# tuna2134/sbv2-api

Measured on AMD Instinct MI355X. Metric: audio_seconds_per_second, higher is better.
Workload: dtype bf16x3-split (decoder + flow convs: bf16 hi/lo MFMA, f32 accumulate/storage) + f16x3 (DeBERTa GEMMs, flow 1x1: f16 hi + scaled f16 lo per operand, 22 mantissa bits, f32 accumulate) + f32 (text side)

## Files before the change

include/sbv2_hip.h:

```cpp
#ifndef SBV2_HIP_H
#define SBV2_HIP_H

#include <stddef.h>
#include <stdint.h>

#ifdef __cplusplus
extern "C" {
#endif

typedef struct sbv2_bert sbv2_bert;
typedef struct sbv2_vits sbv2_vits;
typedef struct sbv2_pipeline sbv2_pipeline;

const char* sbv2_last_error(void);
int sbv2_device_count(void);

int sbv2_bert_create(const uint8_t* model, size_t model_len, int device, sbv2_bert** out);
void sbv2_bert_destroy(sbv2_bert* h);
int64_t sbv2_bert_hidden(const sbv2_bert* h);
int sbv2_bert_gemm_parts(const sbv2_bert* h);

int sbv2_bert_predict(sbv2_bert* h, const int64_t* token_ids, const int64_t* attention_mask, int64_t S, float* out);
int sbv2_bert_predict_batch(sbv2_bert* h, int64_t n, const int64_t* token_ids, const int64_t* attention_mask,
                            const int64_t* lens, float* out);
// ... 354 lines not shown
                           float* ms);
int sbv2_debug_set_skinny_max(int workgroups);
int sbv2_debug_set_clx(int on);
int sbv2_debug_set_ksplit(int on);
int sbv2_debug_set_flash_parts(int on);
int sbv2_debug_conv1d_clx(int device, const float* x, const float* w, const float* bias, const float* res, int64_t cin, int64_t cout, int64_t k,
                          int64_t L, int64_t dilation, float pre_slope, float beta, int64_t iters, float* y, float* ys_sum, float* ms);
int sbv2_debug_f16x3_saturation(int device, int enable, uint64_t* count);
int sbv2_debug_set_respair_clx(int on);
int sbv2_debug_respair(int device, const float* x, const float* w1, const float* w2, const float* b1, const float* b2, int64_t C, int64_t N, int64_t k,
                       int64_t dilation, const uint8_t* mask, int64_t mask_div, float beta, int accumulate, int variant, float* y);
int sbv2_debug_set_resbranch(int on);
int sbv2_debug_set_upx(int on);
int sbv2_debug_conv_transpose1d_clx(int device, const float* x, const float* w, const float* bias, int64_t cin, int64_t cout, int64_t k, int64_t L,
                                    int64_t stride, float pre_slope, const uint8_t* mask, int64_t mask_div, int64_t iters, float* y, float* ys_sum, float* ms);
int sbv2_debug_resbranch(int device, const float* x, const float* w, const float* bias, int64_t C, int64_t N, int64_t k, const int64_t* dilations,
                         const uint8_t* mask, int64_t mask_div, float beta, int accumulate, int variant, int64_t iters, float* y, float* ms);
int sbv2_debug_resbranch_ys(int device, const float* x, const float* w, const float* bias, int64_t C, int64_t N, int64_t k, const int64_t* dilations,
                            const uint8_t* mask, int64_t mask_div, float beta, int accumulate, int64_t iters, float* y, float* ys, float* y_steps, float* ys_steps,
                            float* ms);
int sbv2_debug_gemm_bfs(int device, const float* x, const float* w, const float* bias, const float* res, int64_t M, int64_t N, int64_t K,
                        int parts, int act, int split_out, int64_t iters, float* y, float* ms);
int sbv2_debug_gemm_bfs_alt(int device, const float* xa, const float* xb, const float* w, const float* bias, const float* res, int64_t M, int64_t N, int64_t K,
                            int parts, int64_t iters, float* ya, float* yb);
int sbv2_debug_repeat_respair(int device, const float* xa, const float* xb, const float* w1, const float* w2, const float* b1, const float* b2, int64_t C,
                              int64_t N, int64_t k, int64_t dilation, const uint8_t* mask, int64_t mask_div, float beta, const float* prev, int variant,
                              int reps, int neighbour, int flip_at, int64_t flip_word, float* ya, float* yb, int64_t* mismatch, int64_t* first_bad);
int sbv2_debug_repeat_resbranch(int device, const float* xa, const float* xb, const float* w, const float* bias, int64_t C, int64_t N, int64_t k,
                                const int64_t* dilations, const uint8_t* mask, int64_t mask_div, float beta, const float* prev, int reps, int neighbour,
                                int flip_at, int64_t flip_word, float* ya, float* yb, int64_t* mismatch, int64_t* first_bad);
// ... 77 lines not shown
```

sbv2-api_amd/_lib.py:

```python
import ctypes as C
import os

_HERE = os.path.dirname(os.path.abspath(__file__))
LIB_PATH = os.path.join(_HERE, "libsbv2_hip.so")

i64p = C.POINTER(C.c_int64)
f32p = C.POINTER(C.c_float)


class Sbv2Batch(C.Structure):
    _fields_ = [
        ("n", C.c_int64), ("t_lens", i64p), ("x_tst", i64p), ("tones", i64p), ("lang_ids", i64p), ("sids", i64p),
        ("style_vectors", f32p), ("bert", f32p),
        ("sdp_ratio", C.c_float), ("length_scale", C.c_float), ("noise_scale", C.c_float), ("noise_scale_w", C.c_float),
        ("noise_seed", C.c_uint64), ("forced_durations", i64p),
    ]


class Sbv2PcmFormat(C.Structure):
    _fields_ = [("sample_rate", C.c_int32), ("encoding", C.c_int32), ("normalize", C.c_int32), ("reserved", C.c_int32)]


class Sbv2Loudness(C.Structure):
    _fields_ = [("target_lufs", C.c_double), ("true_peak_max_dbtp", C.c_double)]
# ... 253 lines not shown
    "sbv2_style_vector": (C.c_int, [f32p, C.c_int64, C.c_int64, C.c_int64, C.c_float, f32p]),
    "sbv2_debug_import_to_container": (C.c_int, [C.c_void_p, C.c_size_t, C.c_int, C.POINTER(C.c_void_p), C.POINTER(C.c_size_t)]),
    "sbv2_debug_bucket_table": (C.c_int, [C.c_int64, C.c_int64, C.c_int64, C.POINTER(C.c_int32)]),
    "sbv2_debug_conv1d": (C.c_int, [C.c_int, f32p, f32p, f32p, C.c_int64, C.c_int64, C.c_int64, C.c_int64, C.c_int64, C.c_float, f32p]),
    "sbv2_debug_conv_transpose1d": (C.c_int, [C.c_int, f32p, f32p, f32p, C.c_int64, C.c_int64, C.c_int64, C.c_int64, C.c_int64,
                                              C.c_int64, C.c_float, f32p]),
    "sbv2_debug_conv1d_cl": (C.c_int, [C.c_int, f32p, f32p, f32p, C.c_int64, C.c_int64, C.c_int64, C.c_int64, C.c_int64, C.c_float, C.c_int,
                                       C.c_int64, f32p, f32p]),
    "sbv2_debug_time_conv1d": (C.c_int, [C.c_int, C.c_int64, C.c_int64, C.c_int64, C.c_int64, C.c_int64, C.c_int64, f32p]),
    "sbv2_debug_set_skinny_max": (C.c_int, [C.c_int]),
    "sbv2_debug_set_clx": (C.c_int, [C.c_int]),
    "sbv2_debug_set_ksplit": (C.c_int, [C.c_int]),
    "sbv2_debug_set_flash_parts": (C.c_int, [C.c_int]),
    "sbv2_debug_conv1d_clx": (C.c_int, [C.c_int, f32p, f32p, f32p, f32p, C.c_int64, C.c_int64, C.c_int64, C.c_int64, C.c_int64, C.c_float, C.c_float,
                                        C.c_int64, f32p, f32p, f32p]),
    "sbv2_debug_set_respair_clx": (C.c_int, [C.c_int]),
    "sbv2_debug_f16x3_saturation": (C.c_int, [C.c_int, C.c_int, C.POINTER(C.c_uint64)]),
    "sbv2_debug_respair": (C.c_int, [C.c_int, f32p, f32p, f32p, f32p, f32p, C.c_int64, C.c_int64, C.c_int64, C.c_int64, C.c_void_p, C.c_int64, C.c_float, C.c_int,
                                     C.c_int, f32p]),
    "sbv2_debug_set_resbranch": (C.c_int, [C.c_int]),
    "sbv2_debug_set_upx": (C.c_int, [C.c_int]),
    "sbv2_debug_conv_transpose1d_clx": (C.c_int, [C.c_int, f32p, f32p, f32p, C.c_int64, C.c_int64, C.c_int64, C.c_int64, C.c_int64, C.c_float, C.c_void_p,
                                                  C.c_int64, C.c_int64, f32p, f32p, f32p]),
    "sbv2_debug_resbranch": (C.c_int, [C.c_int, f32p, f32p, f32p, C.c_int64, C.c_int64, C.c_int64, i64p, C.c_void_p, C.c_int64, C.c_float, C.c_int, C.c_int,
                                       C.c_int64, f32p, f32p]),
    "sbv2_debug_resbranch_ys": (C.c_int, [C.c_int, f32p, f32p, f32p, C.c_int64, C.c_int64, C.c_int64, i64p, C.c_void_p, C.c_int64, C.c_float, C.c_int,
                                          C.c_int64, f32p, f32p, f32p, f32p, f32p]),
    "sbv2_debug_gemm_bfs_alt": (C.c_int, [C.c_int, f32p, f32p, f32p, f32p, f32p, C.c_int64, C.c_int64, C.c_int64, C.c_int, C.c_int64, f32p, f32p]),
    "sbv2_debug_repeat_respair": (C.c_int, [C.c_int, f32p, f32p, f32p, f32p, f32p, f32p, C.c_int64, C.c_int64, C.c_int64, C.c_int64, C.c_void_p, C.c_int64,
                                            C.c_float, f32p, C.c_int, C.c_int, C.c_int, C.c_int, C.c_int64, f32p, f32p, i64p, i64p]),
# ... 78 lines not shown
```

sbv2-api_amd/csrc/common.h:

```cpp
#pragma once
#include <hip/hip_runtime.h>

#include <atomic>

#include <cstdint>
#include <cstdio>
#include <map>
#include <memory>
#include <stdexcept>
#include <exception>
#include <string>
#include <vector>

namespace sbv2 {

void set_last_error(const std::string& msg);

struct Error : std::runtime_error {
    using std::runtime_error::runtime_error;
};

#define HIP_CHECK(expr)                                                                          \
    do {                                                                                         \
        hipError_t _e = (expr);                                                                  \
// ... 253 lines not shown
    const unsigned char* mask = nullptr;
    int mask_div = 1;
    int out_stride = 1, phase_rows = 1 << 30;
    int phase_off[kMaxPhases] = {0};
    int in_km = 0, out_km = 0;
    int act = ACT_NONE;
    float alpha = 1.0f;
    void* ys_p = nullptr;
    int64_t ys_rows = 0;
    int ys_front = 0;
    float ys_slope = 1.0f;
};
void launch_conv_cl(const ConvClParams& p, hipStream_t stream);
bool conv_cl_parts_ok(const ConvClParams& p);
bool launch_conv_cl_small(const ConvClParams& p, int mask_shift, hipStream_t stream);

constexpr int kPartsF16x3 = 4;
constexpr float kF16LoScale = 2048.0f;
inline int split_nplanes(int code) { return code == kPartsF16x3 ? 2 : code; }
struct SplitPlanes {
    void* p = nullptr;
    int parts = 0, C = 0, L = 0, ld = 0;
    int f16 = 0;
    int64_t pstride = 0;
    unsigned long long* sat = nullptr;
    int code() const { return f16 ? kPartsF16x3 : parts; }
    SplitPlanes rows(int c0, int n) const {
        SplitPlanes s = *this;
        s.p = static_cast<char*>(p) + (size_t)c0 * ld * 2;
        s.C = n;
// ... 217 lines not shown
```

sbv2-api_amd/csrc/conv_clx.hip:

```cpp
#include <atomic>
#include <type_traits>

#include "common.h"
#include "device_prims.h"

#pragma clang fp contract(off)

namespace sbv2 {

constexpr int kClxNT = 256;
constexpr int kClxXR = 320;

struct ClxKernelParams {
    ConvClxParams p;
    int xrows;
    int wshift0;
    int sh0, sh_step;
    int gy;
};

template <int NTAPS, int kClxWR, int kClxXB, int XR, int EPI, bool PH = false>
__global__ __launch_bounds__(256) __attribute__((amdgpu_waves_per_eu(kClxWR * 4096 + kClxXB * 2 * XR * 32 <= 53 * 1024 ? 3 : 2))) void conv_clx_kernel(const ClxKernelParams kp) {
    constexpr bool EDGE = EPI == 1;
    static_assert(!PH || EPI == 0 || EPI == 3, "phased output: whole-tile channels-last epilogues only");
// ... 297 lines not shown
            int ostride = 1, mch = m;
            int64_t orow = nf16;
            if constexpr (PH) {
                ostride = p.out_stride;
                if (p.phase_group == 2) {
                    const int blk = (m0 >> 5) + i, nb = p.phase_rows >> 4;
                    const int pg = blk / nb;
                    mch = (blk - pg * nb) * 16 + (c8 & 15);
                    orow = (int64_t)nf16 * ostride + p.phase_off[2 * pg] + (c8 >> 4);
                } else {
                    const int ph = m0 / p.phase_rows;
                    mch = m - ph * p.phase_rows;
                    orow = (int64_t)nf16 * ostride + p.phase_off[ph];
                }
            }
            float* yp = p.Y ? p.Y + orow * p.ldy + mch : nullptr;
            const int64_t ystep = (int64_t)16 * ostride * p.ldy;
            const int64_t qstep = (int64_t)512 * ostride;
            char* qs = p.Ys.p ? static_cast<char*>(p.Ys.p) + ((int64_t)(mch >> 4) * 2) * yplane + ((int64_t)p.Ys.front + orow) * 32 + (mch & 15) * 2 : nullptr;
#pragma unroll
            for (int it = 0; it < 4; ++it) {
                f32x4v v[2];
#pragma unroll
                for (int h = 0; h < 2; ++h) {
                    const f32x4v a = *reinterpret_cast<const f32x4v*>(trow8 + it * 16 * 36 + 4 * h);
                    v[h] = a + b8[i][h];
                    if (p.R) v[h] += acc_y ? ld[0][it][h] : ld[i][it][h];
                    v[h] *= beta;
                    if (acc_y) v[h] += ld[1][it][h];
                    if (!allkeep && !((mbits >> it) & 1u)) v[h] = f32x4v{0.f, 0.f, 0.f, 0.f};
                }
// ... 32 lines not shown
        constexpr int i = decltype(ic)::value;
        tile_write(ic);
        const int m = m0 + i * 32 + c4;
        const f32x4v b4 = p.bias ? *reinterpret_cast<const f32x4v*>(p.bias + m) : f32x4v{0.f, 0.f, 0.f, 0.f};
#pragma unroll 1
        for (int it = 0; it < 8; ++it) {
            const int n = nfirst + it * 8;
            const int64_t pp = min(n, N - 1);
            const f32x4v a = *reinterpret_cast<const f32x4v*>(trow + it * 8 * 36);
            f32x4v v = a + b4;
            if (p.R) v += *reinterpret_cast<const f32x4v*>(p.R + pp * p.ldr + m);
            v *= beta;
            if (p.accumulate) v += *reinterpret_cast<const f32x4v*>(p.Y + pp * p.ldy + m);
            if (p.mask && !p.mask[pp >> p.mask_shift]) v = f32x4v{0.f, 0.f, 0.f, 0.f};
            if (n < N) {
                if (p.Y) *reinterpret_cast<f32x4v*>(p.Y + (int64_t)n * p.ldy + m) = v;
                if (p.Ys.p) {
                    char* qs = static_cast<char*>(p.Ys.p) + ((int64_t)(m >> 4) * 2) * yplane + ((int64_t)p.Ys.front + n) * 32 + (m & 15) * 2;
                    bf16x4 h, l;
#pragma unroll
                    for (int e = 0; e < 4; ++e) {
                        const float x = fmaxf(v[e], v[e] * sl);
                        h[e] = (__bf16)x;
                        l[e] = (__bf16)(x - (float)h[e]);
                    }
                    *reinterpret_cast<bf16x4*>(qs) = h;
                    *reinterpret_cast<bf16x4*>(qs + yplane) = l;
                }
            }
        }
    });
// ... 83 lines not shown
    hipLaunchKernelGGL(k_split_cl_km, dim3((unsigned)((x.L + 255) / 256), x.C >> 4), dim3(256), 0, stream, x.p, x.ld, (int64_t)x.L, x.C, slope, out);
    HIP_CHECK(hipGetLastError());
}

bool conv_clx_usable(const ConvClxParams& p) {
    if (!(p.ntaps == 3 || p.ntaps == 5 || p.ntaps == 7 || p.ntaps == 11 || (p.phase_rows && (p.ntaps == 2 || p.ntaps == 4)))) return false;
    if (p.Ykm && (p.Y || p.Ys.p || p.accumulate || p.R)) return false;
    if ((p.K & 31) || (p.M & 63) || p.K != p.X.C) return false;
    int tapmax = p.ntaps - 1;
    if (p.phase_rows)
        for (int q = 0; q < kMaxPhases && q < p.M / std::max(p.phase_rows, 1); ++q) tapmax = std::max(tapmax, p.ntaps - 1 + p.phase_tap0[q]);
    const int span = tapmax * std::abs(p.shift_step);
    if (span > kClxXR - kClxNT || p.shift0 < -kClxFront || p.shift0 + span > 64) return false;
    if (p.mask && p.mask_shift < 0) return false;
    if (p.Y && (p.ldy & 3)) return false;
    if (p.R && (p.ldr & 3)) return false;
    if (p.phase_rows) {
        if ((p.phase_rows & 63) || p.M % p.phase_rows || p.M / p.phase_rows > kMaxPhases || p.out_stride < 1 || p.R || p.accumulate || p.Ykm || p.N < kClxNT ||
            (p.ntaps & 1)) return false;
        if (p.Y && p.ldy < p.phase_rows) return false;
        if (p.Ys.p && (p.Ys.C != p.phase_rows || p.Ys.N != (int64_t)p.N * p.out_stride)) return false;
        for (int q = 0; q < p.M / p.phase_rows; ++q)
            if (p.phase_off[q] < 0 || p.phase_off[q] >= p.out_stride) return false;
        if (p.phase_group == 2) {
            if ((p.M / p.phase_rows) & 1) return false;
            for (int q = 0; q < p.M / p.phase_rows; q += 2)
                if (p.phase_off[q + 1] != p.phase_off[q] + 1 || p.phase_tap0[q + 1] != p.phase_tap0[q]) return false;
        } else if (p.phase_group != 1) return false;
        for (int q = 0; q < p.M / p.phase_rows; ++q)
            if (p.phase_tap0[q] < 0 || p.phase_tap0[q] > 8) return false;
// ... 104 lines not shown
```

sbv2-api_amd/csrc/decoder_cl.cpp:

```cpp
#include <algorithm>
#include <atomic>
#include <cmath>
#include <cstring>

#include "models.h"

namespace sbv2 {

static inline uint16_t f32_to_bf16_rne(float f) {
    uint32_t u;
    std::memcpy(&u, &f, 4);
    if ((u & 0x7FFFFFFFu) > 0x7F800000u) return (uint16_t)((u >> 16) | 0x40);
    u += 0x7FFFu + ((u >> 16) & 1u);
    return (uint16_t)(u >> 16);
}
static inline uint16_t f32_to_f16_rne(float f) {
    uint32_t u;
    std::memcpy(&u, &f, 4);
    const uint32_t sign = (u >> 16) & 0x8000u;
    u &= 0x7FFFFFFFu;
    if (u >= 0x7F800000u) return (uint16_t)(sign | 0x7C00u | (u > 0x7F800000u ? 0x200u : 0u));
    if (u >= 0x477FF000u) return (uint16_t)(sign | 0x7C00u);
    if (u < 0x33000001u) return (uint16_t)sign;
    int e = (int)(u >> 23) - 127;
// ... 154 lines not shown
    u.ntaps = U;
    u.shift0 = -tmin;
    u.nph = s;
    u.cout = cout;
    u.group = group;
    u.alg_macs_per_pos = macs;
    for (int r = 0; r < s; ++r) {
        u.phase_off[r] = r;
        u.phase_tap0[r] = t0[r] - tmin;
    }
    return u;
}

static int cl_parts_of(int mode) { return mode == 1 ? 2 : (mode == 2 ? 1 : 3); }

ClConv pack_decoder_conv(WeightStore& ws, const float* w, int M, int K, int k, int mode, const float* bias) {
    ClConv c = pack_cl(ws, w, M, K, k, cl_parts_of(mode), bias);
    if (mode == 1 && M == 16 && K == 16) c.wp = pack_cl_pairs(ws, w, k);
    return c;
}

void VitsModel::load_decoder_cl(const Blob& blob) {
    auto conv = [&](const std::string& prefix, int mode) {
        const HostTensor& t = blob.get(prefix + ".weight");
        const float* b = blob.has(prefix + ".bias") ? blob.get(prefix + ".bias").data : nullptr;
        return pack_decoder_conv(*ws_, t.data, (int)t.dims[0], (int)t.dims[1], (int)t.dims[2], mode, b);
    };
    std::vector<int> stage_mode(cfg_.up_rates.size(), dec_mode_);
    if (const char* e = getenv("SBV2_DECODER_STAGES")) {
        std::string v(e);
// ... 11 lines not shown
    }
    cl_pre_ = conv("dec.conv_pre", dec_mode_);
    int C = cfg_.up_initial;
    const int nk = (int)cfg_.res_kernels.size();
    for (size_t i = 0; i < cfg_.up_rates.size(); ++i) {
        ClStage st;
        st.mode = stage_mode[i];
        st.rate = cfg_.up_rates[i];
        st.cin = C;
        C /= 2;
        st.ch = C;
        const HostTensor& t = blob.get("dec.ups." + std::to_string(i) + ".weight");
        const float* ub = blob.get("dec.ups." + std::to_string(i) + ".bias").data;
        const int k = (int)t.dims[2], s = st.rate, pad = (k - s) / 2, cin = (int)t.dims[0], cout = (int)t.dims[1];
        SBV2_REQUIRE(k - 2 * pad == s, "transposed conv must upsample exactly by its stride");
        std::vector<std::vector<int>> tsets(s);
        for (int r = 0; r < s; ++r)
            for (int tt = -k; tt <= k; ++tt) {
                const int j = s * tt + r + pad;
                if (j >= 0 && j < k) tsets[r].push_back(tt);
            }
        std::vector<bool> done(s, false);
        for (int r = 0; r < s; ++r) {
            if (done[r]) continue;
            std::vector<int> phases;
            for (int r2 = r; r2 < s && (int)phases.size() < kMaxPhases; ++r2)
                if (!done[r2] && tsets[r2] == tsets[r]) {
                    phases.push_back(r2);
                    done[r2] = true;
                }
            ClUpGroup g;
            g.ntaps = (int)tsets[r].size();
            g.nph = (int)phases.size();
            const int M = g.nph * cout;
            std::vector<float> w((size_t)M * cin * g.ntaps), bias((size_t)M);
            for (int pi = 0; pi < g.nph; ++pi)
                for (int co = 0; co < cout; ++co) {
                    bias[pi * cout + co] = ub[co];
                    for (int ci = 0; ci < cin; ++ci)
                        for (int ti = 0; ti < g.ntaps; ++ti)
                            w[((size_t)(pi * cout + co) * cin + ci) * g.ntaps + ti] =
                                t.data[((size_t)ci * cout + co) * k + (s * tsets[r][ti] + phases[pi] + pad)];
                }
            for (int ti = 0; ti < g.ntaps; ++ti) g.shift[ti] = -tsets[r][ti];
            for (int pi = 0; pi < kMaxPhases; ++pi) g.phase_off[pi] = pi < g.nph ? phases[pi] : 0;
            g.c = pack_cl(*ws_, w.data(), M, cin, g.ntaps, cl_parts_of(st.mode), bias.data());
            st.up.push_back(g);
        }
        if (st.mode == 1 && st.ch >= 64) st.upx = build_upx(*ws_, t.data, ub, cin, cout, k, s, st.ch >= 128);
        for (int j = 0; j < nk; ++j) {
            ClBranch rb;
            rb.k = cfg_.res_kernels[j];
            rb.dil = cfg_.res_dilations[j];
            const std::string p = "dec.resblocks." + std::to_string(i * nk + j) + ".";
            for (size_t n = 0; n < rb.dil.size(); ++n) {
                rb.c1.push_back(conv(p + "convs1." + std::to_string(n), st.mode));
                rb.c2.push_back(conv(p + "convs2." + std::to_string(n), st.mode));
            }
            st.branches.push_back(rb);
        }
        cl_stages_.push_back(st);
    }
}
// ... 102 lines not shown
    p.M = C;
    p.N = (int)N;
    p.K = C;
    p.ntaps = k;
    p.shift0 = -dil * (k - 1) / 2;
    p.shift_step = dil;
    p.Ys = T;
    p.ys_slope = 0.1f;
    p.bias = c1.bias;
    p.mask = mask;
    p.mask_shift = mask_shift;
    return p;
}

ConvClxParams clx_conv2_params(const ClConv& c2, const SplitClPlanes& T, int C, int64_t N, int k, const float* R, float* Y, const SplitClPlanes* Ys, float beta,
                               int accumulate, const unsigned char* mask, int mask_shift) {
    ConvClxParams p;
    p.X = T;
    p.W = c2.wx;
    p.nmt = c2.nmt;
    p.M = C;
    p.N = (int)N;
    p.K = C;
    p.ntaps = k;
    p.shift0 = -(k - 1) / 2;
    p.shift_step = 1;
    p.Y = Y;
    p.ldy = C;
    if (Ys) {
        p.Ys = *Ys;
        p.ys_slope = 0.1f;
    }
    p.bias = c2.bias;
    p.R = R;
    p.ldr = C;
    p.beta = beta;
    p.accumulate = accumulate;
    p.mask = mask;
    p.mask_shift = mask_shift;
    return p;
}

struct VitsModel::ClStagePlan {
    bool upx = false;
    bool upx_in_parts = false;
    bool clx = false;
    bool up_parts = false;
    bool next_parts = false;
    std::vector<BranchKernel> branch;
};

std::vector<VitsModel::ClStagePlan> VitsModel::plan_decoder_cl(int64_t Lf, const unsigned char* mask) const {
    const int clx_mode = read_knob(g_clx, "SBV2_CLX must be 0, 1 or 2"), upx_on = read_knob(g_upx, "SBV2_UPX must be 0 or 1"),
              rb_on = read_knob(g_rb, "SBV2_RESBRANCH must be 0 or 1"), rp_on = g_rpx.load(std::memory_order_relaxed);
    const int nk = (int)cfg_.res_kernels.size();
    auto upx_at = [&](size_t si, int64_t Lin, int Uin) {
        const ClStage& st = cl_stages_[si];
        return clx_mode && upx_on && st.mode == 1 && st.upx.wx && Lin >= 256 && (Uin & (Uin - 1)) == 0 &&
               clx_size_ok(clx_mode, (Lin / 256) * (st.upx.M / 64), 128);
    };
    std::vector<ClStagePlan> plan(cl_stages_.size());
    plan[0].upx = upx_at(0, Lf, 1);
    int64_t Lin = Lf;
// ... 4 lines not shown
        U *= st.rate;
        const int64_t Lo = Lf * U;
        const int C = st.ch;
        const bool pow2 = (U & (U - 1)) == 0;
        int ushift = 0;
        while ((1 << ushift) < U) ++ushift;
        sp.clx = clx_mode && st.mode == 1 && C >= 128 && (C & 63) == 0 && pow2 && clx_size_ok(clx_mode, (Lo / 256) * (C / 64), 128);
        for (const ClBranch& rb : st.branches) {
            if (!(rb.k == 3 || rb.k == 7 || rb.k == 11) || !rb.c1[0].wx) sp.clx = false;
            for (int d : rb.dil)
                if (d * (rb.k - 1) > 64 || d * (rb.k - 1) / 2 > kClxFront) sp.clx = false;
        }
        if (si + 1 < cl_stages_.size()) {
            plan[si + 1].upx = upx_at(si + 1, Lo, U);
            sp.next_parts = plan[si + 1].upx_in_parts = sp.clx && plan[si + 1].upx;
        }
        sp.up_parts = sp.clx;
        if (sp.clx && !sp.upx)
            for (const ClUpGroup& g : st.up) {
                ConvClParams p;
                p.split = 1;
                p.tm = g.c.tm;
                p.nmt = g.c.nmt;
                p.N = (int)Lin;
                sp.up_parts = sp.up_parts && conv_cl_parts_ok(p);
            }
        for (int j = 0; j < nk; ++j) {
            const ClBranch& rb = st.branches[j];
            if (rb_on && ((!sp.clx && C <= 64) || (sp.clx && C == 128)) && st.mode == 1 && (int)rb.dil.size() == kResBranchSteps && pow2 &&
                !(sp.next_parts && j + 1 == nk) && resbranch_usable(branch_params(rb.c1, rb.c2, rb.dil, rb.k, C, Lo, mask, ushift)))
                sp.branch.push_back(BranchKernel::resbranch);
// ... 75 lines not shown
            }
            pu.bias = st.upx.bias;
            pu.mask = fl.d_mask;
            pu.mask_shift = ushift_in;
            pu.out_stride = st.rate;
            pu.phase_rows = C;
            pu.phase_group = st.upx.group;
            for (int q = 0; q < kMaxPhases; ++q) {
                pu.phase_off[q] = st.upx.phase_off[q];
                pu.phase_tap0[q] = st.upx.phase_tap0[q];
            }
            pu.prof_flops = 2.0 * st.upx.alg_macs_per_pos * (double)Lcur;
            launch_conv_clx(pu, stream_);
        } else {
            for (const auto& g : st.up) {
                ConvClParams p;
                p.X = cur;
                p.ldx = st.cin;
                p.NB = (int)Lcur;
                p.W = g.c.w;
                p.nmt = g.c.nmt;
                p.tm = g.c.tm;
                p.split = st.mode == 1;
                p.f16 = st.mode == 3;
                p.M = g.c.M;
                p.N = (int)Lcur;
                p.K = st.cin;
                p.ntaps = g.ntaps;
                for (int t = 0; t < g.ntaps; ++t) p.shift[t] = g.shift[t];
                p.Y = XU;
                p.ldy = C;
                p.bias = g.c.bias;
                p.pre_slope = 0.1f;
                p.mask = fl.d_mask;
                p.mask_div = U;
                p.out_stride = st.rate;
                p.phase_rows = C;
                for (int q = 0; q < kMaxPhases; ++q) p.phase_off[q] = g.phase_off[q];
                if (sp.up_parts) {
                    p.ys_p = XUs.p;
                    p.ys_rows = (int64_t)XUs.front + XUs.N + XUs.back;
                    p.ys_front = XUs.front;
                    p.ys_slope = 0.1f;
                }
                launch_conv_cl(p, stream_);
            }
            if (sp.clx && !sp.up_parts) split_cl(XU, C, Lo, C, 0.1f, XUs, stream_);
        }
        for (int j = 0; j < nk; ++j) {
            const ClBranch& rb = st.branches[j];
            const BranchKernel kern = sp.branch[j];
            const float* y = XU;
            const SplitClPlanes* ys = &XUs;
            const int nd = (int)rb.dil.size();
            if (kern == BranchKernel::resbranch) {
                ResBranchParams bp = branch_params(rb.c1, rb.c2, rb.dil, rb.k, C, Lo, fl.d_mask, ushift);
                bp.X = XU;
                bp.Y = XS;
                bp.beta = 1.0f / nk;
                bp.accumulate = j > 0;
                launch_resbranch(bp, stream_);
                continue;
            }
            for (int q = 0; q < nd; ++q) {
                const int d = rb.dil[q];
                const bool last = q + 1 == nd;
                float* yn = last ? XS : ((y == YA) ? YB : YA);
                if (kern == BranchKernel::clx_steps) {
                    launch_conv_clx(clx_conv1_params(rb.c1[q], *ys, T1s, C, Lo, rb.k, d, fl.d_mask, ushift), stream_);
                    const SplitClPlanes* yns = (ys == &YsA) ? &YsB : &YsA;
                    const SplitClPlanes* out_parts = !last ? yns : (sp.next_parts && j + 1 == nk ? &XSs : nullptr);
                    launch_conv_clx(clx_conv2_params(rb.c2[q], T1s, C, Lo, rb.k, y, yn, out_parts, last ? 1.0f / nk : 1.0f, last && j > 0, fl.d_mask, ushift),
                                    stream_);
                    ys = yns;
                } else if (kern == BranchKernel::conv_cl_steps) {
                    conv_cl(rb.c1[q], y, C, (int)Lo, T1, C, (int)Lo, d, d * (rb.k - 1) / 2, fl.d_mask, U, 0.1f, nullptr, 0, 1.0f, 0);
                    conv_cl(rb.c2[q], T1, C, (int)Lo, yn, C, (int)Lo, 1, (rb.k - 1) / 2, fl.d_mask, U, 0.1f, y, C, last ? 1.0f / nk : 1.0f,
                            last && j > 0);
                } else {
                    ResPairParams rp = step_params(rb.c1[q], rb.c2[q], rb.k, d, st.mode, C, Lo, fl.d_mask, U, ushift);
                    rp.X = y;
                    rp.Y = yn;
                    rp.beta = last ? 1.0f / nk : 1.0f;
                    rp.accumulate = last && j > 0;
                    launch_respair(rp, kern, stream_);
                }
                y = yn;
            }
        }
        ar.rewind(mk);
        cur = XS;
        Lcur = Lo;
        cur_s = XSs;
    }
    pcm_lens_.assign(n, 0);
    pcm_offs_.assign(n, 0);
    int64_t tot = 0, maxlen = 0;
    for (int u = 0; u < n; ++u) {
        pcm_offs_[u] = tot;
        pcm_lens_[u] = (int64_t)fl.len[u] * U;
        tot += pcm_lens_[u];
        maxlen = std::max(maxlen, pcm_lens_[u]);
    }
    pcm_total_ = tot;
    pcm_ = ar.array<float>((size_t)tot);
    int64_t* d_off = ar.array<int64_t>(n);
// ... 6 lines not shown
```

sbv2-api_amd/csrc/models.h:

```cpp
#pragma once
#include "common.h"
#include "flac_encode.h"
#include "limiter.h"
#include "marks.h"
#include "ops.h"
#include "pcm_format.h"
#include "stream_output.h"

#include <memory>

namespace sbv2 {

struct ClConv {
    void* w = nullptr;
    void* wxp = nullptr;
    void* wx = nullptr;
    void* wp = nullptr;
    float* bias = nullptr;
    int M = 0, K = 0, k = 1, nmt = 0, tm = 1, parts = 0;
};

struct PackedConv {
    float* w = nullptr;
    float* bias = nullptr;
// ... 30 lines not shown
SegLayout make_layout(const std::vector<int>& lens, int gap, Arena& arena, hipStream_t stream, const unsigned char* extra_mask = nullptr, int round_to = 4);

class WeightStore;
ClConv pack_cl(WeightStore& ws, const float* w, int M, int K, int k, int parts, const float* bias);
void* pack_clx16(WeightStore& ws, const float* w, int M, int K, int k);
struct ClUpX {
    void* wx = nullptr;
    float* bias = nullptr;
    int M = 0, K = 0, ntaps = 0, shift0 = 0, nph = 0, cout = 0;
    int group = 1;
    double alg_macs_per_pos = 0;
    int phase_off[kMaxPhases] = {0};
    int phase_tap0[kMaxPhases] = {0};
};
ClUpX build_upx(WeightStore& ws, const float* wt, const float* ub, int cin, int cout, int k, int s, bool parts_out);
void* pack_step_pairs(WeightStore& ws, const float* w, int C, int k);
void* pack_cl_pairs(WeightStore& ws, const float* w, int k);
ClConv pack_decoder_conv(WeightStore& ws, const float* w, int M, int K, int k, int mode, const float* bias);
ConvClParams conv_cl_params(const ClConv& c, const float* X, int ldx, int NB, float* Y, int ldy, int N, int dil, int pad_l, const unsigned char* mask,
                            int mask_div, float pre_slope, const float* R, int ldr, float beta, int accumulate);
ResPairParams step_params(const ClConv& c1, const ClConv& c2, int k, int dil, int mode, int C, int64_t N, const unsigned char* mask, int U, int ushift);
ResBranchParams branch_params(const std::vector<ClConv>& c1, const std::vector<ClConv>& c2, const std::vector<int>& dil, int k, int C, int64_t N,
                              const unsigned char* mask, int mask_shift);
ConvClxParams clx_conv1_params(const ClConv& c1, const SplitClPlanes& X, const SplitClPlanes& T, int C, int64_t N, int k, int dil, const unsigned char* mask,
                               int mask_shift);
ConvClxParams clx_conv2_params(const ClConv& c2, const SplitClPlanes& T, int C, int64_t N, int k, const float* R, float* Y, const SplitClPlanes* Ys, float beta,
                               int accumulate, const unsigned char* mask, int mask_shift);
BfsWeights pack_bfs(WeightStore& ws, const float* w, int M, int K, int parts);

class WeightStore {
  public:
    explicit WeightStore(const Blob& b, int cl_parts = 0) : blob_(b), cl_parts_(cl_parts) {}
    int cl_parts() const { return cl_parts_; }
    void set_cl_parts(int parts) { cl_parts_ = parts; }
    int bfs_parts() const { return bfs_parts_; }
    void set_bfs_parts(int parts) { bfs_parts_ = parts; }
    ~WeightStore();
    float* upload(const float* host, size_t n);
    float* tensor(const std::string& name);
    float* tensor(const std::string& name, std::initializer_list<int64_t> dims);
    void expect(const PackedConv& c, const std::string& prefix, int cout, int cin, int k) const;
    PackedConv conv(const std::string& prefix, bool bias = true);
// ... 254 lines not shown
        PackedUpsample up;
        std::vector<ResBranch> branches;
        int ch, rate;
    };
    struct TraceEntry {
        Plane p;
        const SegLayout* lay;
        int div;
    };

    Encoder load_encoder(const std::string& prefix, int n_layers);
    DDS load_dds(const std::string& prefix, int channels);
    void run_encoder(const Encoder& e, Plane x, const SegLayout& lay, const float* spk_vec, Arena& ar);
    void run_dds(const DDS& d, Plane x, const SegLayout& lay, Arena& ar);
    void run_decoder(Arena& ar, Plane z, const SegLayout& fl, const float* cond_vec);
    struct ClUpGroup {
        ClConv c;
        int ntaps = 0, nph = 0;
        int shift[kMaxTaps];
        int phase_off[kMaxPhases];
    };
    struct ClBranch {
        std::vector<ClConv> c1, c2;
        std::vector<int> dil;
        int k;
    };
    struct ClStage {
        std::vector<ClUpGroup> up;
        ClUpX upx;
        std::vector<ClBranch> branches;
        int cin, ch, rate;
        int mode = 1;
    };
    struct ClStagePlan;
    void load_decoder_cl(const Blob& blob);
    std::vector<ClStagePlan> plan_decoder_cl(int64_t Lf, const unsigned char* mask) const;
// ... 76 lines not shown
```

sbv2-api_amd/csrc/ops.hip:

```cpp
#include "ops.h"

#include <cfloat>

namespace sbv2 {

__device__ __forceinline__ float wave_sum(float v) {
#pragma unroll
    for (int o = 32; o > 0; o >>= 1) v += __shfl_xor(v, o, 64);
    return v;
}
__device__ __forceinline__ float gelu_exact(float v) { return 0.5f * v * (1.0f + erff(v * 0.70710678118654752440f)); }

__global__ __launch_bounds__(256) void k_deberta_embed_ln(const int* ids, const float* emb, int H, const float* gamma,
                                                           const float* beta, float eps, Plane out) {
    __shared__ float red[4];
    const int n = blockIdx.x;
    const int id = ids[n];
    const int tid = threadIdx.x;
    if (id < 0) {
        for (int c = tid; c < H; c += 256) out.p[(size_t)c * out.ld + n] = 0.f;
        return;
    }
    const float* row = emb + (size_t)id * H;
    float s = 0.f;
// ... 804 lines not shown
    } else {
        v = make_float4(0.f, 0.f, 0.f, 0.f);
    }
    *p = v;
}
void add_segvec_cl(float* x, int L, int C, const float* vec, int vec_ld, const int* seg_of, const unsigned char* mask, hipStream_t s) {
    const int64_t n4 = (int64_t)L * (C >> 2);
    hipLaunchKernelGGL(k_add_segvec_cl, dim3((unsigned)((n4 + 255) / 256)), dim3(256), 0, s, x, L, C, vec, vec_ld, seg_of, mask);
}

constexpr int kPostMaxC = 32, kPostMaxK = 12;
template <int CT, int KT>
__global__ __launch_bounds__(256) void k_conv_post_tanh_cl(const float* x, int C_, int64_t L, const float* w, int k_, float slope,
                                                            const int* seg_start, const int* seg_len, const int64_t* pcm_off, int up,
                                                            float* pcm) {
    __shared__ float xs[(256 + kPostMaxK) * (kPostMaxC + 4)];
    __shared__ float ws[kPostMaxC * kPostMaxK];
    const int C = CT > 0 ? CT : C_, k = KT > 0 ? KT : k_;
    const int sg = blockIdx.y;
    const int64_t len = (int64_t)seg_len[sg] * up;
    const int64_t s0 = (int64_t)blockIdx.x * 256;
    if (s0 >= len) return;
    const int tid = threadIdx.x;
    const int half = k / 2;
    const int pitch = C + 4;
    const int c4n = C >> 2;
    const int64_t row0 = (int64_t)seg_start[sg] * up + s0 - half;
    for (int idx = tid; idx < (256 + k - 1) * c4n; idx += 256) {
        const int r = idx / c4n, c4 = idx - r * c4n;
        const int64_t q = row0 + r;
        float4 v = make_float4(0.f, 0.f, 0.f, 0.f);
        if (q >= 0 && q < L) v = *reinterpret_cast<const float4*>(x + q * C + c4 * 4);
// ... 82 lines not shown
```

Measured before the change: 5041.

## Add dedicated one-tap upsample kernel and skip fp32 output when only parts needed

Adds a specialized kernel for one-tap split-bf16 transposed convolutions (64->2x32, 32->2x16) that keeps weights in registers, applies leaky-relu and hi/lo bf16 split inline, and writes phase-interleaved output via LDS transpose with nontemporal stores. When the next stage consumes only split bf16 parts, the last resblock conv2 now skips writing the fp32 output (accumulate mode 2), saving a full-precision store. Also shrinks static shared memory of the post conv for templated sizes to improve occupancy. This adds new code paths and eligibility checks that must match the existing layouts.

Measured after the change: 4847. 3.9% lower.

```diff
diff --git a/include/sbv2_hip.h b/include/sbv2_hip.h
--- a/include/sbv2_hip.h
+++ b/include/sbv2_hip.h
@@ -392,6 +392,10 @@
 int sbv2_debug_set_upx(int on);
 int sbv2_debug_conv_transpose1d_clx(int device, const float* x, const float* w, const float* bias, int64_t cin, int64_t cout, int64_t k, int64_t L,
                                     int64_t stride, float pre_slope, const uint8_t* mask, int64_t mask_div, int64_t iters, float* y, float* ys_sum, float* ms);
+int sbv2_debug_conv_transpose1d_cl(int device, const float* x, const float* w, const float* bias, int64_t cin, int64_t cout, int64_t k, int64_t L,
+                                   int64_t stride, const uint8_t* mask, int64_t mask_div, int kernel, float* y);
+int sbv2_debug_conv2_clx_sum(int device, const float* t, const float* w, const float* bias, const float* res, const float* prev, int64_t C, int64_t N,
+                             int64_t k, const uint8_t* mask, int64_t mask_div, float beta, int parts_only, float* y, uint16_t* parts);
 int sbv2_debug_resbranch(int device, const float* x, const float* w, const float* bias, int64_t C, int64_t N, int64_t k, const int64_t* dilations,
                          const uint8_t* mask, int64_t mask_div, float beta, int accumulate, int variant, int64_t iters, float* y, float* ms);
 int sbv2_debug_resbranch_ys(int device, const float* x, const float* w, const float* bias, int64_t C, int64_t N, int64_t k, const int64_t* dilations,
diff --git a/sbv2-api_amd/_lib.py b/sbv2-api_amd/_lib.py
--- a/sbv2-api_amd/_lib.py
+++ b/sbv2-api_amd/_lib.py
@@ -291,6 +291,10 @@
     "sbv2_debug_set_flash_parts": (C.c_int, [C.c_int]),
     "sbv2_debug_conv1d_clx": (C.c_int, [C.c_int, f32p, f32p, f32p, f32p, C.c_int64, C.c_int64, C.c_int64, C.c_int64, C.c_int64, C.c_float, C.c_float,
                                         C.c_int64, f32p, f32p, f32p]),
+    "sbv2_debug_conv_transpose1d_cl": (C.c_int, [C.c_int, f32p, f32p, f32p, C.c_int64, C.c_int64, C.c_int64, C.c_int64, C.c_int64, C.c_void_p, C.c_int64,
+                                                 C.c_int, f32p]),
+    "sbv2_debug_conv2_clx_sum": (C.c_int, [C.c_int, f32p, f32p, f32p, f32p, f32p, C.c_int64, C.c_int64, C.c_int64, C.c_void_p, C.c_int64, C.c_float, C.c_int,
+                                           f32p, C.c_void_p]),
     "sbv2_debug_set_respair_clx": (C.c_int, [C.c_int]),
     "sbv2_debug_f16x3_saturation": (C.c_int, [C.c_int, C.c_int, C.POINTER(C.c_uint64)]),
     "sbv2_debug_respair": (C.c_int, [C.c_int, f32p, f32p, f32p, f32p, f32p, C.c_int64, C.c_int64, C.c_int64, C.c_int64, C.c_void_p, C.c_int64, C.c_float, C.c_int,
diff --git a/sbv2-api_amd/csrc/common.h b/sbv2-api_amd/csrc/common.h
--- a/sbv2-api_amd/csrc/common.h
+++ b/sbv2-api_amd/csrc/common.h
@@ -291,6 +291,8 @@
 void launch_conv_cl(const ConvClParams& p, hipStream_t stream);
 bool conv_cl_parts_ok(const ConvClParams& p);
 bool launch_conv_cl_small(const ConvClParams& p, int mask_shift, hipStream_t stream);
+bool upx1_cl_usable(const ConvClParams& p);
+void launch_upx1_cl(const ConvClParams& p, hipStream_t stream);
 
 constexpr int kPartsF16x3 = 4;
 constexpr float kF16LoScale = 2048.0f;
diff --git a/sbv2-api_amd/csrc/conv_clx.hip b/sbv2-api_amd/csrc/conv_clx.hip
--- a/sbv2-api_amd/csrc/conv_clx.hip
+++ b/sbv2-api_amd/csrc/conv_clx.hip
@@ -335,7 +335,7 @@
                     orow = (int64_t)nf16 * ostride + p.phase_off[ph];
                 }
             }
-            float* yp = p.Y ? p.Y + orow * p.ldy + mch : nullptr;
+            float* yp = p.Y && p.accumulate != 2 ? p.Y + orow * p.ldy + mch : nullptr;
             const int64_t ystep = (int64_t)16 * ostride * p.ldy;
             const int64_t qstep = (int64_t)512 * ostride;
             char* qs = p.Ys.p ? static_cast<char*>(p.Ys.p) + ((int64_t)(mch >> 4) * 2) * yplane + ((int64_t)p.Ys.front + orow) * 32 + (mch & 15) * 2 : nullptr;
@@ -398,7 +398,7 @@
             if (p.accumulate) v += *reinterpret_cast<const f32x4v*>(p.Y + pp * p.ldy + m);
             if (p.mask && !p.mask[pp >> p.mask_shift]) v = f32x4v{0.f, 0.f, 0.f, 0.f};
             if (n < N) {
-                if (p.Y) *reinterpret_cast<f32x4v*>(p.Y + (int64_t)n * p.ldy + m) = v;
+                if (p.Y && p.accumulate != 2) *reinterpret_cast<f32x4v*>(p.Y + (int64_t)n * p.ldy + m) = v;
                 if (p.Ys.p) {
                     char* qs = static_cast<char*>(p.Ys.p) + ((int64_t)(m >> 4) * 2) * yplane + ((int64_t)p.Ys.front + n) * 32 + (m & 15) * 2;
                     bf16x4 h, l;
@@ -512,6 +512,7 @@
     if (span > kClxXR - kClxNT || p.shift0 < -kClxFront || p.shift0 + span > 64) return false;
     if (p.mask && p.mask_shift < 0) return false;
     if (p.Y && (p.ldy & 3)) return false;
+    if (p.accumulate < 0 || p.accumulate > 2 || (p.accumulate && !p.Y) || (p.accumulate == 2 && !p.Ys.p)) return false;
     if (p.R && (p.ldr & 3)) return false;
     if (p.phase_rows) {
         if ((p.phase_rows & 63) || p.M % p.phase_rows || p.M / p.phase_rows > kMaxPhases || p.out_stride < 1 || p.R || p.accumulate || p.Ykm || p.N < kClxNT ||
diff --git a/sbv2-api_amd/csrc/decoder_cl.cpp b/sbv2-api_amd/csrc/decoder_cl.cpp
--- a/sbv2-api_amd/csrc/decoder_cl.cpp
+++ b/sbv2-api_amd/csrc/decoder_cl.cpp
@@ -192,6 +192,72 @@
 
 static int cl_parts_of(int mode) { return mode == 1 ? 2 : (mode == 2 ? 1 : 3); }
 
+std::vector<ClUpGroup> build_up_groups(WeightStore& ws, const float* wt, const float* ub, int cin, int cout, int k, int s, int mode) {
+    const int pad = (k - s) / 2;
+    std::vector<ClUpGroup> up;
+    std::vector<std::vector<int>> tsets(s);
+    for (int r = 0; r < s; ++r)
+        for (int tt = -k; tt <= k; ++tt) {
+            const int j = s * tt + r + pad;
+            if (j >= 0 && j < k) tsets[r].push_back(tt);
+        }
+    std::vector<bool> done(s, false);
+    for (int r = 0; r < s; ++r) {
+        if (done[r]) continue;
+        std::vector<int> phases;
+        for (int r2 = r; r2 < s && (int)phases.size() < kMaxPhases; ++r2)
+            if (!done[r2] && tsets[r2] == tsets[r]) {
+                phases.push_back(r2);
+                done[r2] = true;
+            }
+        ClUpGroup g;
+        g.ntaps = (int)tsets[r].size();
+        g.nph = (int)phases.size();
+        const int M = g.nph * cout;
+        std::vector<float> w((size_t)M * cin * g.ntaps), bias((size_t)M);
+        for (int pi = 0; pi < g.nph; ++pi)
+            for (int co = 0; co < cout; ++co) {
+                bias[pi * cout + co] = ub[co];
+                for (int ci = 0; ci < cin; ++ci)
+                    for (int ti = 0; ti < g.ntaps; ++ti)
+                        w[((size_t)(pi * cout + co) * cin + ci) * g.ntaps + ti] = wt[((size_t)ci * cout + co) * k + (s * tsets[r][ti] + phases[pi] + pad)];
+            }
+        for (int ti = 0; ti < g.ntaps; ++ti) g.shift[ti] = -tsets[r][ti];
+        for (int pi = 0; pi < kMaxPhases; ++pi) g.phase_off[pi] = pi < g.nph ? phases[pi] : 0;
+        g.c = pack_cl(ws, w.data(), M, cin, g.ntaps, cl_parts_of(mode), bias.data());
+        up.push_back(g);
+    }
+    return up;
+}
+
+ConvClParams up_group_params(const ClUpGroup& g, int mode, const float* X, int cin, int64_t Lin, float* Y, int cout, int s, const unsigned char* mask,
+                             int mask_div) {
+    ConvClParams p;
+    p.X = X;
+    p.ldx = cin;
+    p.NB = (int)Lin;
+    p.W = g.c.w;
+    p.nmt = g.c.nmt;
+    p.tm = g.c.tm;
+    p.split = mode == 1;
+    p.f16 = mode == 3;
+    p.M = g.c.M;
+    p.N = (int)Lin;
+    p.K = cin;
+    p.ntaps = g.ntaps;
+    for (int t = 0; t < g.ntaps; ++t) p.shift[t] = g.shift[t];
+    p.Y = Y;
+    p.ldy = cout;
+    p.bias = g.c.bias;
+    p.pre_slope = 0.1f;
+    p.mask = mask;
+    p.mask_div = mask_div;
+    p.out_stride = s;
+    p.phase_rows = cout;
+    for (int q = 0; q < kMaxPhases; ++q) p.phase_off[q] = g.phase_off[q];
+    return p;
+}
+
 ClConv pack_decoder_conv(WeightStore& ws, const float* w, int M, int K, int k, int mode, const float* bias) {
     ClConv c = pack_cl(ws, w, M, K, k, cl_parts_of(mode), bias);
     if (mode == 1 && M == 16 && K == 16) c.wp = pack_cl_pairs(ws, w, k);
@@ -233,39 +299,7 @@
         const float* ub = blob.get("dec.ups." + std::to_string(i) + ".bias").data;
         const int k = (int)t.dims[2], s = st.rate, pad = (k - s) / 2, cin = (int)t.dims[0], cout = (int)t.dims[1];
         SBV2_REQUIRE(k - 2 * pad == s, "transposed conv must upsample exactly by its stride");
-        std::vector<std::vector<int>> tsets(s);
-        for (int r = 0; r < s; ++r)
-            for (int tt = -k; tt <= k; ++tt) {
-                const int j = s * tt + r + pad;
-                if (j >= 0 && j < k) tsets[r].push_back(tt);
-            }
-        std::vector<bool> done(s, false);
-        for (int r = 0; r < s; ++r) {
-            if (done[r]) continue;
-            std::vector<int> phases;
-            for (int r2 = r; r2 < s && (int)phases.size() < kMaxPhases; ++r2)
-                if (!done[r2] && tsets[r2] == tsets[r]) {
-                    phases.push_back(r2);
-                    done[r2] = true;
-                }
-            ClUpGroup g;
-            g.ntaps = (int)tsets[r].size();
-            g.nph = (int)phases.size();
-            const int M = g.nph * cout;
-            std::vector<float> w((size_t)M * cin * g.ntaps), bias((size_t)M);
-            for (int pi = 0; pi < g.nph; ++pi)
-                for (int co = 0; co < cout; ++co) {
-                    bias[pi * cout + co] = ub[co];
-                    for (int ci = 0; ci < cin; ++ci)
-                        for (int ti = 0; ti < g.ntaps; ++ti)
-                            w[((size_t)(pi * cout + co) * cin + ci) * g.ntaps + ti] =
-                                t.data[((size_t)ci * cout + co) * k + (s * tsets[r][ti] + phases[pi] + pad)];
-                }
-            for (int ti = 0; ti < g.ntaps; ++ti) g.shift[ti] = -tsets[r][ti];
-            for (int pi = 0; pi < kMaxPhases; ++pi) g.phase_off[pi] = pi < g.nph ? phases[pi] : 0;
-            g.c = pack_cl(*ws_, w.data(), M, cin, g.ntaps, cl_parts_of(st.mode), bias.data());
-            st.up.push_back(g);
-        }
+        st.up = build_up_groups(*ws_, t.data, ub, cin, cout, k, s, st.mode);
         if (st.mode == 1 && st.ch >= 64) st.upx = build_upx(*ws_, t.data, ub, cin, cout, k, s, st.ch >= 128);
         for (int j = 0; j < nk; ++j) {
             ClBranch rb;
@@ -398,7 +432,7 @@
 }
 
 ConvClxParams clx_conv2_params(const ClConv& c2, const SplitClPlanes& T, int C, int64_t N, int k, const float* R, float* Y, const SplitClPlanes* Ys, float beta,
-                               int accumulate, const unsigned char* mask, int mask_shift) {
+                               int accumulate, const unsigned char* mask, int mask_shift, bool parts_only) {
     ConvClxParams p;
     p.X = T;
     p.W = c2.wx;
@@ -409,7 +443,7 @@
     p.ntaps = k;
     p.shift0 = -(k - 1) / 2;
     p.shift_step = 1;
-    p.Y = Y;
+    p.Y = parts_only && !accumulate ? nullptr : Y;
     p.ldy = C;
     if (Ys) {
         p.Ys = *Ys;
@@ -419,7 +453,7 @@
     p.R = R;
     p.ldr = C;
     p.beta = beta;
-    p.accumulate = accumulate;
+    p.accumulate = accumulate ? (parts_only ? 2 : 1) : 0;
     p.mask = mask;
     p.mask_shift = mask_shift;
     return p;
@@ -427,10 +461,12 @@
 
 struct VitsModel::ClStagePlan {
     bool upx = false;
+    bool upx1 = false;
     bool upx_in_parts = false;
     bool clx = false;
     bool up_parts = false;
     bool next_parts = false;
+    bool sum_parts_only = false;
     std::vector<BranchKernel> branch;
 };
 
@@ -465,7 +501,11 @@
         if (si + 1 < cl_stages_.size()) {
             plan[si + 1].upx = upx_at(si + 1, Lo, U);
             sp.next_parts = plan[si + 1].upx_in_parts = sp.clx && plan[si + 1].upx;
-        }
+            sp.sum_parts_only = sp.next_parts;
+        }
+        if (!sp.upx && st.up.size() == 1)
+            sp.upx1 = upx1_cl_usable(up_group_params(st.up[0], st.mode, nullptr, st.cin, Lin, nullptr, C, st.rate, mask, U)) &&
+                      clx_size_ok(clx_mode, Lin / 256, 2048);
         sp.up_parts = sp.clx;
         if (sp.clx && !sp.upx)
             for (const ClUpGroup& g : st.up) {
@@ -571,36 +611,15 @@
             launch_conv_clx(pu, stream_);
         } else {
             for (const auto& g : st.up) {
-                ConvClParams p;
-                p.X = cur;
-                p.ldx = st.cin;
-                p.NB = (int)Lcur;
-                p.W = g.c.w;
-                p.nmt = g.c.nmt;
-                p.tm = g.c.tm;
-                p.split = st.mode == 1;
-                p.f16 = st.mode == 3;
-                p.M = g.c.M;
-                p.N = (int)Lcur;
-                p.K = st.cin;
-                p.ntaps = g.ntaps;
-                for (int t = 0; t < g.ntaps; ++t) p.shift[t] = g.shift[t];
-                p.Y = XU;
-                p.ldy = C;
-                p.bias = g.c.bias;
-                p.pre_slope = 0.1f;
-                p.mask = fl.d_mask;
-                p.mask_div = U;
-                p.out_stride = st.rate;
-                p.phase_rows = C;
-                for (int q = 0; q < kMaxPhases; ++q) p.phase_off[q] = g.phase_off[q];
+                ConvClParams p = up_group_params(g, st.mode, cur, st.cin, Lcur, XU, C, st.rate, fl.d_mask, U);
                 if (sp.up_parts) {
                     p.ys_p = XUs.p;
                     p.ys_rows = (int64_t)XUs.front + XUs.N + XUs.back;
                     p.ys_front = XUs.front;
                     p.ys_slope = 0.1f;
                 }
-                launch_conv_cl(p, stream_);
+                if (sp.upx1) launch_upx1_cl(p, stream_);
+                else launch_conv_cl(p, stream_);
             }
             if (sp.clx && !sp.up_parts) split_cl(XU, C, Lo, C, 0.1f, XUs, stream_);
         }
@@ -627,7 +646,9 @@
                     launch_conv_clx(clx_conv1_params(rb.c1[q], *ys, T1s, C, Lo, rb.k, d, fl.d_mask, ushift), stream_);
                     const SplitClPlanes* yns = (ys == &YsA) ? &YsB : &YsA;
                     const SplitClPlanes* out_parts = !last ? yns : (sp.next_parts && j + 1 == nk ? &XSs : nullptr);
-                    launch_conv_clx(clx_conv2_params(rb.c2[q], T1s, C, Lo, rb.k, y, yn, out_parts, last ? 1.0f / nk : 1.0f, last && j > 0, fl.d_mask, ushift),
+                    const bool parts_only = sp.sum_parts_only && out_parts == &XSs;
+                    launch_conv_clx(clx_conv2_params(rb.c2[q], T1s, C, Lo, rb.k, y, yn, out_parts, last ? 1.0f / nk : 1.0f, last && j > 0, fl.d_mask, ushift,
+                                                     parts_only),
                                     stream_);
                     ys = yns;
                 } else if (kern == BranchKernel::conv_cl_steps) {
@@ -646,7 +667,7 @@
             }
         }
         ar.rewind(mk);
-        cur = XS;
+        cur = sp.sum_parts_only ? nullptr : XS;
         Lcur = Lo;
         cur_s = XSs;
     }
diff --git a/sbv2-api_amd/csrc/models.h b/sbv2-api_amd/csrc/models.h
--- a/sbv2-api_amd/csrc/models.h
+++ b/sbv2-api_amd/csrc/models.h
@@ -68,6 +68,15 @@
     int phase_tap0[kMaxPhases] = {0};
 };
 ClUpX build_upx(WeightStore& ws, const float* wt, const float* ub, int cin, int cout, int k, int s, bool parts_out);
+struct ClUpGroup {
+    ClConv c;
+    int ntaps = 0, nph = 0;
+    int shift[kMaxTaps];
+    int phase_off[kMaxPhases];
+};
+std::vector<ClUpGroup> build_up_groups(WeightStore& ws, const float* wt, const float* ub, int cin, int cout, int k, int s, int mode);
+ConvClParams up_group_params(const ClUpGroup& g, int mode, const float* X, int cin, int64_t Lin, float* Y, int cout, int s, const unsigned char* mask,
+                             int mask_div);
 void* pack_step_pairs(WeightStore& ws, const float* w, int C, int k);
 void* pack_cl_pairs(WeightStore& ws, const float* w, int k);
 ClConv pack_decoder_conv(WeightStore& ws, const float* w, int M, int K, int k, int mode, const float* bias);
@@ -79,7 +88,7 @@
 ConvClxParams clx_conv1_params(const ClConv& c1, const SplitClPlanes& X, const SplitClPlanes& T, int C, int64_t N, int k, int dil, const unsigned char* mask,
                                int mask_shift);
 ConvClxParams clx_conv2_params(const ClConv& c2, const SplitClPlanes& T, int C, int64_t N, int k, const float* R, float* Y, const SplitClPlanes* Ys, float beta,
-                               int accumulate, const unsigned char* mask, int mask_shift);
+                               int accumulate, const unsigned char* mask, int mask_shift, bool parts_only = false);
 BfsWeights pack_bfs(WeightStore& ws, const float* w, int M, int K, int parts);
 
 class WeightStore {
@@ -364,12 +373,6 @@
     void run_encoder(const Encoder& e, Plane x, const SegLayout& lay, const float* spk_vec, Arena& ar);
     void run_dds(const DDS& d, Plane x, const SegLayout& lay, Arena& ar);
     void run_decoder(Arena& ar, Plane z, const SegLayout& fl, const float* cond_vec);
-    struct ClUpGroup {
-        ClConv c;
-        int ntaps = 0, nph = 0;
-        int shift[kMaxTaps];
-        int phase_off[kMaxPhases];
-    };
     struct ClBranch {
         std::vector<ClConv> c1, c2;
         std::vector<int> dil;
diff --git a/sbv2-api_amd/csrc/ops.hip b/sbv2-api_amd/csrc/ops.hip
--- a/sbv2-api_amd/csrc/ops.hip
+++ b/sbv2-api_amd/csrc/ops.hip
@@ -842,8 +842,8 @@
 __global__ __launch_bounds__(256) void k_conv_post_tanh_cl(const float* x, int C_, int64_t L, const float* w, int k_, float slope,
                                                             const int* seg_start, const int* seg_len, const int64_t* pcm_off, int up,
                                                             float* pcm) {
-    __shared__ float xs[(256 + kPostMaxK) * (kPostMaxC + 4)];
-    __shared__ float ws[kPostMaxC * kPostMaxK];
+    __shared__ float xs[(256 + (KT > 0 ? KT : kPostMaxK)) * ((CT > 0 ? CT : kPostMaxC) + 4)];
+    __shared__ float ws[CT > 0 ? 1 : kPostMaxC * kPostMaxK];
     const int C = CT > 0 ? CT : C_, k = KT > 0 ? KT : k_;
     const int sg = blockIdx.y;
     const int64_t len = (int64_t)seg_len[sg] * up;
diff --git a/sbv2-api_amd/csrc/upx1_cl.hip b/sbv2-api_amd/csrc/upx1_cl.hip
--- /dev/null
+++ b/sbv2-api_amd/csrc/upx1_cl.hip
@@ -0,0 +1,168 @@
+#include <algorithm>
+
+#include "common.h"
+#include "device_prims.h"
+
+#pragma clang fp contract(off)
+
+namespace sbv2 {
+
+constexpr int kUx1NT = 256;
+constexpr int kUx1MaxGrid = 2048;
+
+struct Upx1KernelParams {
+    const float* X;
+    int ldx;
+    int N;
+    const void* W;
+    const float* bias;
+    float* Y;
+    const unsigned char* mask;
+    int mask_nshift;
+    float slope;
+    int phase_rows;
+    int ntiles;
+};
+
+template <int KC, int TM>
+__global__ __launch_bounds__(256) void upx1_cl_kernel(const Upx1KernelParams p) {
+    constexpr int M = TM * 32;
+    __shared__ __attribute__((aligned(16))) float tiles[4][64 * 36];
+    const int tid = threadIdx.x, lane = tid & 63;
+    const int wave = __builtin_amdgcn_readfirstlane(tid >> 6);
+    const int lcol = lane & 31, lh = lane >> 5;
+    const int N = p.N;
+
+    bf16x8 ah[KC][TM], al[KC][TM];
+#pragma unroll
+    for (int c = 0; c < KC; ++c)
+#pragma unroll
+        for (int i = 0; i < TM; ++i) {
+            const char* blk = static_cast<const char*>(p.W) + ((c * TM + i) * 2) * 1024 + lane * 16;
+            ah[c][i] = *reinterpret_cast<const bf16x8*>(blk);
+            al[c][i] = *reinterpret_cast<const bf16x8*>(blk + 1024);
+        }
+    const int c4 = (lane & 7) * 4, prow = lane >> 3;
+    f32x4v b4[TM];
+#pragma unroll
+    for (int i = 0; i < TM; ++i) {
+        const int m = i * 32 + c4;
+        b4[i] = p.bias ? *reinterpret_cast<const f32x4v*>(p.bias + (m - (m / p.phase_rows) * p.phase_rows)) : f32x4v{0.f, 0.f, 0.f, 0.f};
+    }
+    float* tile = tiles[wave];
+    const float slope = p.slope;
+
+    for (int t = blockIdx.x; t < p.ntiles; t += gridDim.x) {
+        const int nw = t * kUx1NT + wave * 64;
+        if (nw >= N) continue;
+        f32x4v rx[2][KC][2];
+#pragma unroll
+        for (int j = 0; j < 2; ++j) {
+            const float* row = p.X + (int64_t)min(nw + j * 32 + lcol, N - 1) * p.ldx + 8 * lh;
+#pragma unroll
+            for (int c = 0; c < KC; ++c) {
+                rx[j][c][0] = *reinterpret_cast<const f32x4v*>(row + c * 16);
+                rx[j][c][1] = *reinterpret_cast<const f32x4v*>(row + c * 16 + 4);
+            }
+        }
+        const unsigned char* mp = p.mask ? p.mask + (min(nw + lane, N - 1) >> p.mask_nshift) : reinterpret_cast<const unsigned char*>(p.X);
+        const unsigned mraw = *mp;
+        const unsigned mv = p.mask ? mraw : 1u;
+        f32x16 acc[TM][2];
+#pragma unroll
+        for (int i = 0; i < TM; ++i)
+#pragma unroll
+            for (int j = 0; j < 2; ++j)
+#pragma unroll
+                for (int r = 0; r < 16; ++r) acc[i][j][r] = 0.f;
+#pragma unroll
+        for (int c = 0; c < KC; ++c)
+#pragma unroll
+            for (int j = 0; j < 2; ++j) {
+                bf16x8 bh, bl;
+#pragma unroll
+                for (int e = 0; e < 8; ++e) {
+                    float v = rx[j][c][e >> 2][e & 3];
+                    if (slope != 1.0f) v = v >= 0.f ? v : v * slope;
+                    bh[e] = (__bf16)v;
+                    bl[e] = (__bf16)(v - (float)bh[e]);
+                }
+#pragma unroll
+                for (int i = 0; i < TM; ++i) {
+                    acc[i][j] = mfma32(al[c][i], bh, acc[i][j]);
+                    acc[i][j] = mfma32(ah[c][i], bl, acc[i][j]);
+                    acc[i][j] = mfma32(ah[c][i], bh, acc[i][j]);
+                }
+            }
+        const unsigned long long keep = __builtin_amdgcn_ballot_w64(mv != 0);
+#pragma unroll
+        for (int i = 0; i < TM; ++i) {
+#pragma unroll
+            for (int j = 0; j < 2; ++j)
+#pragma unroll
+                for (int q = 0; q < 4; ++q) {
+                    const f32x4v v = {acc[i][j][4 * q], acc[i][j][4 * q + 1], acc[i][j][4 * q + 2], acc[i][j][4 * q + 3]};
+                    *reinterpret_cast<f32x4v*>(tile + (j * 32 + lcol) * 36 + 8 * q + 4 * lh) = v;
+                }
+            float* yp = p.Y + (int64_t)(nw + prow) * M + i * 32 + c4;
+#pragma unroll
+            for (int it = 0; it < 8; ++it) {
+                const f32x4v a = *reinterpret_cast<const f32x4v*>(tile + (prow + it * 8) * 36 + c4);
+                f32x4v v = a + b4[i];
+                if (!((keep >> (prow + it * 8)) & 1ull)) v = f32x4v{0.f, 0.f, 0.f, 0.f};
+                if (nw + prow + it * 8 < N) __builtin_nontemporal_store(v, reinterpret_cast<f32x4v*>(yp + (int64_t)it * 8 * M));
+            }
+        }
+    }
+}
+
+bool upx1_cl_usable(const ConvClParams& p) {
+    if (!p.split || p.f16 || p.in_km || p.out_km || p.ntaps != 1 || p.shift[0] != 0) return false;
+    if (!((p.K == 64 && p.M == 64) || (p.K == 32 && p.M == 32)) || p.nmt != p.M / 32) return false;
+    if (p.N < 1 || p.NB != p.N || (p.ldx & 3) || p.ldx < p.K) return false;
+    if (p.R || p.accumulate || p.beta != 1.0f || p.alpha != 1.0f || p.act != ACT_NONE || p.ys_p) return false;
+    if (p.phase_rows < 16 || (p.phase_rows & 15) || p.M % p.phase_rows || p.out_stride != p.M / p.phase_rows || p.out_stride > kMaxPhases ||
+        p.ldy != p.phase_rows) return false;
+    for (int q = 0; q < p.out_stride; ++q)
+        if (p.phase_off[q] != q) return false;
+    if (p.mask) {
+        const int os = p.out_stride;
+        if (p.mask_div < 1 || (p.mask_div & (p.mask_div - 1)) || (os & (os - 1)) || p.mask_div % os) return false;
+    }
+    return (int64_t)p.N * p.out_stride < (1ll << 31);
+}
+
+void launch_upx1_cl(const ConvClParams& p, hipStream_t stream) {
+    SBV2_REQUIRE(upx1_cl_usable(p), "upx1_cl: not a one-tap split-bf16 transposed convolution of 64 -> 2 x 32 or 32 -> 2 x 16 channels");
+    Upx1KernelParams kp;
+    kp.X = p.X;
+    kp.ldx = p.ldx;
+    kp.N = p.N;
+    kp.W = p.W;
+    kp.bias = p.bias;
+    kp.Y = p.Y;
+    kp.mask = p.mask;
+    kp.mask_nshift = 0;
+    if (p.mask)
+        while ((p.out_stride << kp.mask_nshift) < p.mask_div) ++kp.mask_nshift;
+    kp.slope = p.pre_slope;
+    kp.phase_rows = p.phase_rows;
+    kp.ntiles = (p.N + kUx1NT - 1) / kUx1NT;
+    const dim3 grid((unsigned)std::min(kp.ntiles, kUx1MaxGrid));
+    hipEvent_t e0 = nullptr, e1 = nullptr;
+    const bool prof = conv_prof_active();
+    if (prof) {
+        HIP_CHECK(hipEventCreate(&e0));
+        HIP_CHECK(hipEventCreate(&e1));
+        HIP_CHECK(hipEventRecord(e0, stream));
+    }
+    if (p.K == 64) hipLaunchKernelGGL((upx1_cl_kernel<4, 2>), grid, dim3(256), 0, stream, kp);
+    else hipLaunchKernelGGL((upx1_cl_kernel<2, 1>), grid, dim3(256), 0, stream, kp);
+    HIP_CHECK(hipGetLastError());
+    if (prof) {
+        HIP_CHECK(hipEventRecord(e1, stream));
+        conv_prof_add(p.M == 64 ? 8 : 9, 2.0 * p.M * (double)p.N * p.K, e0, e1);
+    }
+}
+
+}
```
